# MerlinPCarson/WakeWord-Detection

Hardware: NVIDIA B200
Metric: audio_hours_per_sec (higher is better)
Workload: dtype f16x2->f32

## Files before the change

wakeword_detection_b200/csrc/wavenet_tc.cu:

```cuda
#include <string.h>

#include "wavenet_tc.cuh"

namespace wwb {


struct WnSmem {
  unsigned char U[WN_UBUF];
  float4 skip[8 * WN_ROWS];
  unsigned char W[WN_WST][WN_WBLK];
  WnHead head;
  uint64_t bar_gate[WN_NT], bar_rs[WN_NT], bar_det[WN_NT];
  uint64_t bar_u[WN_NT];
  uint64_t bar_dq[WN_NT];
  uint64_t bar_g[WN_NT];
  uint64_t wfull[WN_WST];
  uint32_t tmem_base;
  int zmax[2][WN_G][2];
  int zcnt[2];
};


#ifdef WWB_WN_DBG2
#define WN_DBG2(k, ev) do { if (P.dbg && blockIdx.x == 0 && grp == (int64_t)gridDim.x) P.dbg[WN_DBG_ROLES * 48 * 4 + 64 + (k) * 16 + (ev)] = clock64(); } while (0)
#else
#define WN_DBG2(k, ev) do { } while (0)
#endif
#ifdef WWB_TIMELINE
#define WN_DBG(role, k, ev) do { if (P.dbg && blockIdx.x == 0 && (grp == (int64_t)gridDim.x || grp == 2 * (int64_t)gridDim.x)) P.dbg[((role) * 48 + (k) + (grp == (int64_t)gridDim.x ? 0 : 24)) * 4 + (ev)] = clock64(); } while (0)
#else
#define WN_DBG(role, k, ev) do { } while (0)
#endif


__device__ __forceinline__ void epi_bar_sync() { asm volatile("bar.sync 1, %0;" ::"n"(WN_EPI_THREADS) : "memory"); }

#ifdef WWB_HANG_DEBUG
#define WN_SPIN_LIMIT (1u << 21)
#define WN_HANG_BASE 4096
__device__ __noinline__ void wn_hang(long long* dbg, int warp, int id, int hk, int hi, uint32_t n_u, uint32_t hx) {
  if (dbg && (threadIdx.x & 31) == 0) {
    long long* base = dbg + WN_HANG_BASE + ((long long)blockIdx.x * 32 + warp) * 8;
    base[0] = id; base[1] = hk; base[2] = hi; base[3] = n_u; base[4] = hx; base[5] = clock64();
  }
  asm volatile("exit;");
}
#define WN_BOUNDED(cond, id) do { uint32_t sp_ = 0; while (!(cond)) if (++sp_ > WN_SPIN_LIMIT) wn_hang(P.dbg, warp, id, hk, hi, n_u, hx); } while (0)
#define WN_MBAR_WAIT(bar, par, id) WN_BOUNDED(mbar_try_wait(bar, par), id)
#define WN_SPIN(bar, par, id) WN_BOUNDED(mbar_test_wait(bar, par), id)
#define WN_HSET(var, val) var = (val)
#else
#define WN_MBAR_WAIT(bar, par, id) mbar_wait(bar, par)
#define WN_SPIN(bar, par, id) mbar_spin(bar, par)
#define WN_HSET(var, val) do { } while (0)
#endif
__device__ __forceinline__ void mbar_spin(uint64_t* bar, uint32_t parity) {
#pragma unroll 1
  while (!mbar_test_wait(bar, parity)) { }
}
#define WN_WAIT_E(bar, par, id) WN_MBAR_WAIT(bar, par, id)
#ifndef WWB_WN_ISS_SUSPEND
#define WN_WAIT_I(bar, par, id) WN_SPIN(bar, par, id)
#else
#define WN_WAIT_I(bar, par, id) WN_MBAR_WAIT(bar, par, id)
#endif

__global__ void __launch_bounds__(WN_THREADS, 1) wavenet_tc_kernel(const WnTcParams P) {
  extern __shared__ __align__(128) unsigned char smem_raw[];
  WnSmem& sm = *reinterpret_cast<WnSmem*>(smem_raw);
  const int tid = threadIdx.x, lane = tid & 31;
  const int warp = __shfl_sync(0xffffffffu, tid >> 5, 0);
  const int64_t n_win = P.wm.n_win_dev ? (int64_t)*P.wm.n_win_dev : P.wm.n_win;
  const int64_t n_groups = P.stream_mode ? P.wm.n_streams * (int64_t)P.chunks_per_stream : (n_win + WN_G - 1) / WN_G;
  const int L = P.L;

  for (int i = tid; i < (int)(sizeof(sm.U) / 16); i += WN_THREADS) reinterpret_cast<uint4*>(sm.U)[i] = make_uint4(0, 0, 0, 0);
  for (int i = tid; i < (int)(sizeof(WnHead) / 16); i += WN_THREADS)
    reinterpret_cast<uint4*>(&sm.head)[i] = reinterpret_cast<const uint4*>(P.head)[i];
  if (tid < 2 * WN_G * 2) (&sm.zmax[0][0][0])[tid] = WN_KEY_NEG_INF;
  if (tid < 2) sm.zcnt[tid] = 0;
  if (tid == 0) {
    for (int i = 0; i < WN_NT; ++i) {
      mbar_init(&sm.bar_u[i], i == 0 ? 5 : 4); mbar_init(&sm.bar_g[i], 4); mbar_init(&sm.bar_gate[i], 1); mbar_init(&sm.bar_rs[i], 1);
      mbar_init(&sm.bar_det[i], 1); mbar_init(&sm.bar_dq[i], 4);
    }
    for (int s = 0; s < WN_WST; ++s) mbar_init(&sm.wfull[s], 1);
    mbar_fence_init();
  }
  if (warp == WN_EPI_WARPS) tmem_alloc(&sm.tmem_base, 512);
  fence_async_smem();
  fence_before_sync();
  __syncthreads();
  fence_after_sync();
  const uint32_t tmem = sm.tmem_base;
  const int nsplit = P.nsplit;
  const uint32_t idesc_gate = make_idesc_f16(128, 32), idesc_rs = make_idesc_f16(128, 48);

  if (warp < WN_EPI_WARPS) {
    const int tile = warp >> 2, q = warp & 3;
    const int o = tile * 128 + q * 32 + lane;
    const int R = P.rstride;
    const int t = o / R, w = o - t * R;
    const uint32_t tacc = tmem + tile * WN_TMEM_TILE;
    const uint32_t tbase = tacc + ((uint32_t)(q * 32) << 16);
    uint32_t n_gate = 0, n_rs = 0, n_u = 0;
#ifdef WWB_HANG_DEBUG
    int hk = -1, hi = tile; uint32_t hx = 0;
#endif
    unsigned char* const Urow = sm.U + (WN_PAD + o) * 16;
    float4* const sk = sm.skip + o;
    {
      uint32_t one[16];
#pragma unroll
      for (int i = 0; i < 16; ++i) one[i] = 0u;
      one[0] = 0x3c003c00u;
      tmem_st16(tmem + ((uint32_t)(q * 32) << 16) + WN_C_ONE, one);
      tmem_st_wait();
    }
    const u64 ZERO2 = pk(0.f, 0.f), ONE2 = pk(1.f, 1.f);
    const int jn = P.join[tile];
    const int src_slot = P.src_slot[tile];
    const bool stream_mode = P.stream_mode != 0;

    u64 x[8];
    bool valid = false, snap_out = false;
    int64_t b = 0;
    float* snap_dst = nullptr;
    auto fetch_state = [&](int64_t g) {
      bool vn = g < n_groups;
      int64_t row = 0;
      snap_out = false;
      if (stream_mode) {
        const int64_t s0 = g / P.chunks_per_stream;
        const int c = (int)(g - s0 * P.chunks_per_stream);
        const int f = c * WN_CHUNK_STEP + o;
        vn = vn && f < P.wm.ring;
        row = s0 * P.wm.ring + (vn ? f : 0);
        snap_out = vn && (c == 0 || o >= WN_CHUNK_WARM);
        snap_dst = P.snap + row * 4;
      } else {
        b = g * WN_G + w;
        vn = vn && (t < L) && (b < n_win);
        int64_t s0 = 0;
        int start = 0;
        if (vn) win_origin(P.wm, b, s0, start);
        int rr = start + (vn ? t : 0);
        if (rr >= P.wm.ring) rr -= P.wm.ring;
        row = s0 * P.wm.ring + rr;
      }
      valid = vn;
      if (src_slot >= 0) {
        const float4* p = reinterpret_cast<const float4*>(P.snap) + (int64_t)src_slot * (WN_SNAP_F / 4) * P.n_rows + row;
#pragma unroll
        for (int i = 0; i < 4; ++i) {
          const float4 v = vn ? __ldg(p + (int64_t)i * P.n_rows) : make_float4(0.f, 0.f, 0.f, 0.f);
          x[2 * i] = pk(v.x, v.y);
          x[2 * i + 1] = pk(v.z, v.w);
        }
#pragma unroll
        for (int i = 0; i < 8; ++i) sk[i * WN_ROWS] = vn ? __ldg(p + (int64_t)(4 + i) * P.n_rows) : make_float4(0.f, 0.f, 0.f, 0.f);
      } else {
        const float4* p = reinterpret_cast<const float4*>(P.x0) + row;
#pragma unroll
        for (int i = 0; i < 4; ++i) {
          const float4 v = vn ? __ldg(p + (int64_t)i * P.n_rows) : make_float4(0.f, 0.f, 0.f, 0.f);
          x[2 * i] = pk(v.x, v.y);
          x[2 * i + 1] = pk(v.z, v.w);
        }
#pragma unroll
        for (int i = 0; i < 8; ++i) sk[i * WN_ROWS] = make_float4(0.f, 0.f, 0.f, 0.f);
      }
    };
    auto put_start_state = [&]() {
      uint32_t ur[16];
#pragma unroll
      for (int i = 0; i < 8; ++i) split2(x[i], ur[i], ur[8 + i]);
      if (valid) {
        *reinterpret_cast<uint4*>(Urow) = make_uint4(ur[0], ur[1], ur[2], ur[3]);
        *reinterpret_cast<uint4*>(Urow + WN_PU) = make_uint4(ur[4], ur[5], ur[6], ur[7]);
        *reinterpret_cast<uint4*>(Urow + 2 * WN_PU) = make_uint4(ur[8], ur[9], ur[10], ur[11]);
        *reinterpret_cast<uint4*>(Urow + 3 * WN_PU) = make_uint4(ur[12], ur[13], ur[14], ur[15]);
      }
      tmem_st16(tbase + WN_C_U, ur);
      tmem_st_wait();
      fence_before_sync();
      fence_async_smem();
      __syncwarp();
      if (lane == 0) mbar_arrive(&sm.bar_u[tile]);
    };
    fetch_state(blockIdx.x);
    if ((int64_t)blockIdx.x < n_groups) put_start_state();
    for (int64_t grp = blockIdx.x; grp < n_groups; grp += gridDim.x, ++n_u) {
      const bool valid_g = valid;
      const bool snap_g = snap_out;
      float* const snap_g_dst = snap_dst;
      for (int k = jn; k < 24; ++k) {
        WN_HSET(hk, k);
        WN_WAIT_E(&sm.bar_gate[tile], n_gate & 1, 5);
        ++n_gate;
        fence_after_sync();
        if (q == 0 && lane == 0) WN_DBG(tile, k, 0);
        if (tile == 0 && q == 0 && lane == 0) WN_DBG2(k, 0);
        {
#pragma unroll
          for (int h8 = 0; h8 < 2; ++h8) {
            float v[16];
            tmem_ld16(tbase + h8 * 16, v);
            tmem_ld_wait();
            if (h8 == 0 && tile == 0 && q == 0 && lane == 0) WN_DBG2(k, 1);
            uint32_t gh[4], gl[4];
#pragma unroll
            for (int p = 0; p < 4; ++p) {
              const float a0 = v[2 * p], a1 = v[2 * p + 1], b0 = v[8 + 2 * p], b1 = v[8 + 2 * p + 1];
              const float ea0 = ex2_approx(fminf(a0, 30.f)), ea1 = ex2_approx(fminf(a1, 30.f));
              const float eb0 = ex2_approx(fminf(b0, 30.f)), eb1 = ex2_approx(fminf(b1, 30.f));
              const u64 tt = fadd2(pk(eb0, eb1), ONE2);
              float d0, d1;
              upk(ffma2(pk(ea0, ea1), tt, tt), d0, d1);
              const float rp = rcp_approx(d0 * d1);
              const float r0 = rp * d1, r1 = rp * d0;
              const u64 g = pk(fmaf(-ea0, r0, r0), fmaf(-ea1, r1, r1));
              split2(g, gh[p], gl[p]);
            }
            tmem_st4(tbase + WN_C_G + h8 * 4, gh);
            tmem_st4(tbase + WN_C_G + 8 + h8 * 4, gl);
          }
          if (tile == 0 && q == 0 && lane == 0) WN_DBG2(k, 2);
          tmem_st_wait();
          if (tile == 0 && q == 0 && lane == 0) WN_DBG2(k, 3);
        }
        fence_before_sync();
        if (q == 0 && lane == 0) WN_DBG(tile, k, 1);
        __syncwarp();
        if (lane == 0) mbar_arrive(&sm.bar_g[tile]);
        if (tile == 0 && q == 0 && lane == 0) WN_DBG2(k, 4);

        WN_WAIT_E(&sm.bar_rs[tile], n_rs & 1, 6);
        ++n_rs;
        fence_after_sync();
        if (q == 0 && lane == 0) WN_DBG(tile, k, 2);
        if (tile == 0 && q == 0 && lane == 0) WN_DBG2(k, 5);
        const bool last = (k == 23);
        if (!last) {
#pragma unroll
          for (int h8 = 0; h8 < 2; ++h8) {
            float r[8];
            tmem_ld8(tbase + WN_C_R + h8 * 8, r);
            tmem_ld_wait();
            uint32_t uh[4], ul[4];
#pragma unroll
            for (int p = 0; p < 4; ++p) {
              const int c = h8 * 4 + p;
              x[c] = add_relu2(x[c], pk(r[2 * p], r[2 * p + 1]));
              split2(x[c], uh[p], ul[p]);
            }
            if (valid_g) {
              *reinterpret_cast<uint4*>(Urow + h8 * WN_PU) = make_uint4(uh[0], uh[1], uh[2], uh[3]);
              *reinterpret_cast<uint4*>(Urow + (2 + h8) * WN_PU) = make_uint4(ul[0], ul[1], ul[2], ul[3]);
            }
            tmem_st4(tbase + WN_C_U + h8 * 4, uh);
            tmem_st4(tbase + WN_C_U + 8 + h8 * 4, ul);
          }
          if (tile == 0 && q == 0 && lane == 0) WN_DBG2(k, 6);
          tmem_st_wait();
          if (tile == 0 && q == 0 && lane == 0) WN_DBG2(k, 8);
          fence_before_sync();
          fence_async_smem();
          __syncwarp();
          if (lane == 0) mbar_arrive(&sm.bar_u[tile]);
          if (q == 0 && lane == 0) WN_DBG(tile, k, 3);
          if (tile == 0 && q == 0 && lane == 0) WN_DBG2(k, 9);
        }
#pragma unroll
        for (int h8 = 0; h8 < 4; ++h8) {
          float s[8];
          tmem_ld8(tbase + WN_C_R + 16 + h8 * 8, s);
          const float4 c0 = sk[(2 * h8) * WN_ROWS], c1 = sk[(2 * h8 + 1) * WN_ROWS];
          tmem_ld_wait();
          const u64 n0 = add_relu2(pk(c0.x, c0.y), pk(s[0], s[1])), n1 = add_relu2(pk(c0.z, c0.w), pk(s[2], s[3]));
          const u64 n2 = add_relu2(pk(c1.x, c1.y), pk(s[4], s[5])), n3 = add_relu2(pk(c1.z, c1.w), pk(s[6], s[7]));
          float4 o0, o1;
          upk(n0, o0.x, o0.y); upk(n1, o0.z, o0.w); upk(n2, o1.x, o1.y); upk(n3, o1.z, o1.w);
          sk[(2 * h8) * WN_ROWS] = o0;
          sk[(2 * h8 + 1) * WN_ROWS] = o1;
          if (last) {
            uint32_t eh[4], el[4];
            split2(relu2(n0), eh[0], el[0]); split2(relu2(n1), eh[1], el[1]);
            split2(relu2(n2), eh[2], el[2]); split2(relu2(n3), eh[3], el[3]);
            const uint32_t cx = tbase + (h8 < 2 ? WN_C_U : WN_C_G) + (h8 & 1) * 4;
            tmem_st4(cx, eh);
            tmem_st4(cx + 8, el);
          }
        }
        fence_before_sync();
        if (stream_mode) {
          const int sl = P.snap_slot[k];
          if (sl >= 0 && snap_g) {
            float4* dst = reinterpret_cast<float4*>(snap_g_dst) + (int64_t)sl * (WN_SNAP_F / 4) * P.n_rows;
#pragma unroll
            for (int i = 0; i < 4; ++i) {
              float a0, a1, a2, a3;
              upk(x[2 * i], a0, a1);
              upk(x[2 * i + 1], a2, a3);
              dst[(int64_t)i * P.n_rows] = make_float4(a0, a1, a2, a3);
            }
#pragma unroll
            for (int i = 0; i < 8; ++i) dst[(int64_t)(4 + i) * P.n_rows] = sk[i * WN_ROWS];
          }
        }
        if (last) {
          tmem_st_wait();
          fence_before_sync();
          __syncwarp();
          if (lane == 0) mbar_arrive(&sm.bar_dq[tile]);
          if (q == 0 && lane == 0) WN_DBG(tile, k, 3);
        }
      }

      if (P.enc_out && valid_g) {
        float4* dst = reinterpret_cast<float4*>(P.enc_out + ((grp * WN_G + w) * L + t) * 32);
#pragma unroll
        for (int n = 0; n < 8; ++n) dst[n] = sk[n * WN_ROWS];
      }
      if (tile == 0 && q == 0 && lane == 0) WN_DBG(WN_NT + 1, 20, 0);
      WN_HSET(hk, 24);
      fetch_state(grp + gridDim.x);
      WN_MBAR_WAIT(&sm.bar_det[tile], n_u & 1, 8);
      fence_after_sync();
      if (tile == 0 && q == 0 && lane == 0) WN_DBG(WN_NT + 1, 20, 1);
      float z0, z1;
      {
        u64 acc0[2] = {pk(0.f, 0.f), pk(0.f, 0.f)}, acc1[2] = {pk(0.f, 0.f), pk(0.f, 0.f)};
#pragma unroll
        for (int h8 = 0; h8 < 4; ++h8) {
          float d[8];
          tmem_ld8(tbase + WN_C_R + h8 * 8, d);
          tmem_ld_wait();
#pragma unroll
          for (int p = 0; p < 4; ++p) {
            const int c = h8 * 8 + 2 * p;
            const u64 e = relu2(fadd2(pk(d[2 * p], d[2 * p + 1]), pk(P.det1_b[c], P.det1_b[c + 1])));
            acc0[p & 1] = ffma2(pk(P.det2_w[c], P.det2_w[c + 1]), e, acc0[p & 1]);
            acc1[p & 1] = ffma2(pk(P.det2_w[32 + c], P.det2_w[32 + c + 1]), e, acc1[p & 1]);
          }
        }
        float fa, fb;
        upk(fadd2(acc0[0], acc0[1]), fa, fb);
        z0 = (fa + fb) + P.det2_b[0];
        upk(fadd2(acc1[0], acc1[1]), fa, fb);
        z1 = (fa + fb) + P.det2_b[1];
      }
      const int zp = (int)(n_u & 1);
      if (!stream_mode) {
#pragma unroll
        for (int dw = 0; dw < WN_G; ++dw) {
          const bool mine = valid_g && (w == dw);
          const unsigned m = __ballot_sync(0xffffffffu, mine);
          if (m) {
            const int k0 = __reduce_max_sync(0xffffffffu, mine ? f2key(z0) : WN_KEY_NEG_INF);
            const int k1 = __reduce_max_sync(0xffffffffu, mine ? f2key(z1) : WN_KEY_NEG_INF);
            if (lane == 0) {
              atomicMax(&sm.zmax[zp][dw][0], k0);
              atomicMax(&sm.zmax[zp][dw][1], k1);
            }
          }
        }
        if (tile == 0 && q == 0 && lane == 0) WN_DBG(WN_NT + 1, 20, 2);
        if (lane == 0) {
          __threadfence_block();
          if (atomicAdd(&sm.zcnt[zp], 1) == WN_EPI_WARPS - 1) {
            __threadfence_block();
            for (int dw = 0; dw < WN_G; ++dw) {
              const int64_t bb = grp * WN_G + dw;
              const float a0 = key2f(sm.zmax[zp][dw][0]), a1 = key2f(sm.zmax[zp][dw][1]);
              sm.zmax[zp][dw][0] = WN_KEY_NEG_INF;
              sm.zmax[zp][dw][1] = WN_KEY_NEG_INF;
              if (bb < n_win) {
                const float m = fmaxf(a0, a1);
                const float e0 = expf(a0 - m), e1 = expf(a1 - m), sden = e0 + e1;
                if (P.det_out) { P.det_out[bb * 2] = e0 / sden; P.det_out[bb * 2 + 1] = e1 / sden; }
                if (P.post) P.post[bb] = e1 / sden;
              }
            }
            sm.zcnt[zp] = 0;
          }
        }
        __syncwarp();
      }
      put_start_state();
      if (tile == 0 && q == 0 && lane == 0) WN_DBG(WN_NT + 1, 20, 3);
    }
  } else if (warp == WN_EPI_WARPS) {
    uint32_t n_u = 0;
#ifdef WWB_HANG_DEBUG
    int hk = -1, hi = -1; uint32_t hx = 0;
#endif
    const uint64_t dU = make_desc(smem_u32(sm.U), WN_PU, 128);
    const uint64_t dWg = make_desc(smem_u32(sm.W[0]), 512, 128);
    const uint64_t dBg = make_desc(smem_u32(sm.W[0]) + WN_OFF_GBIAS, 512, 128);
    const uint64_t dH = make_desc(smem_u32(sm.head.det1_B), 512, 128);
    uint32_t my_groups = 0;
    for (int64_t grp = blockIdx.x; grp < n_groups; grp += gridDim.x) ++my_groups;
    const uint32_t total_loads = my_groups * 24;
    for (uint32_t n = 0; n < (uint32_t)WN_WST && n < total_loads; ++n)
      if (lane == 0) {
        mbar_arrive_expect_tx(&sm.wfull[n], WN_WBLK);
        bulk_g2s(sm.W[n], P.wblob + (size_t)n * WN_WBLK, WN_WBLK, &sm.wfull[n]);
      }
    uint32_t n_w = 0;
    uint32_t cu[WN_NT];
#pragma unroll
    for (int i = 0; i < WN_NT; ++i) cu[i] = 0;
    const uint32_t rs3 = (uint32_t)P.rstride;
    for (int64_t grp = blockIdx.x; grp < n_groups; grp += gridDim.x, ++n_u) {
      for (int k = 0; k < 24; ++k, ++n_w) {
        WN_MBAR_WAIT(&sm.wfull[n_w % WN_WST], (n_w / WN_WST) & 1, 1);
        const uint32_t d = (uint32_t)P.dil[k] * rs3;
        const uint64_t wofs = (uint64_t)((n_w % WN_WST) * (WN_WBLK >> 4));
        const uint64_t b0 = dWg + wofs, bb = dBg + wofs;
#pragma unroll
        for (int i = 0; i < WN_NT; ++i) {
          if (k < P.join[i]) continue;
          WN_HSET(hk, k); WN_HSET(hi, i);
          if (i == 1) WN_DBG(WN_NT + 1, k, 0);
          if (i == 0 && lane == 0) WN_DBG2(k, 10);
          WN_WAIT_I(&sm.bar_u[i], cu[i] & 1, 2);
          ++cu[i];
          if (i == 0 && lane == 0) WN_DBG2(k, 11);
          if (i == 1) WN_DBG(WN_NT + 1, k, 1);
          fence_after_sync();
          if (elect_one()) {
            const uint32_t tacc = tmem + i * WN_TMEM_TILE;
            const uint64_t a0 = dU + (uint64_t)(WN_PAD + i * 128 - 2 * d), a1 = dU + (uint64_t)(WN_PAD + i * 128 - d);
            const uint64_t lo_a = (uint64_t)((2 * WN_PU) >> 4), lo_b = (uint64_t)(3072 >> 4);
            mma_f16_ss(tacc, a0, b0, idesc_gate, false);
            if (nsplit == 3) {
              mma_f16_ss(tacc, a0 + lo_a, b0, idesc_gate, true);
              mma_f16_ss(tacc, a0, b0 + lo_b, idesc_gate, true);
            }
            mma_f16_ss(tacc, a1, b0 + 64, idesc_gate, true);
            if (nsplit == 3) {
              mma_f16_ss(tacc, a1 + lo_a, b0 + 64, idesc_gate, true);
              mma_f16_ss(tacc, a1, b0 + 64 + lo_b, idesc_gate, true);
            }
            mma_f16_ts(tacc, tacc + WN_C_U, b0 + 128, idesc_gate, true);
            if (nsplit == 3) {
              mma_f16_ts(tacc, tacc + WN_C_U + 8, b0 + 128, idesc_gate, true);
              mma_f16_ts(tacc, tacc + WN_C_U, b0 + 128 + lo_b, idesc_gate, true);
            }
            mma_f16_ts(tacc, tmem + WN_C_ONE, bb, idesc_gate, true);
            mma_commit(&sm.bar_gate[i]);
            if (i == 0) WN_DBG2(k, 12);
            if (i == 0) WN_DBG(WN_NT, k, 0);
            if (i == WN_NT - 1) WN_DBG(WN_NT, k, 1);
          }
          __syncwarp();
          if (i == 1) WN_DBG(WN_NT + 1, k, 2);
        }
        auto refill = [&](uint32_t m) {
          const uint32_t nl = m + WN_WST;
          if (nl < total_loads && lane == 0) {
            mbar_arrive_expect_tx(&sm.wfull[nl % WN_WST], WN_WBLK);
            bulk_g2s(sm.W[nl % WN_WST], P.wblob + (size_t)(nl % 24) * WN_WBLK, WN_WBLK, &sm.wfull[nl % WN_WST]);
          }
        };
        if (n_w >= 1) refill(n_w - 1);
      }
#pragma unroll
      for (int i = 0; i < WN_NT; ++i) {
        WN_MBAR_WAIT(&sm.bar_dq[i], n_u & 1, 9);
        fence_after_sync();
        if (elect_one()) {
          const uint32_t tacc = tmem + i * WN_TMEM_TILE;
#pragma unroll
          for (int kk = 0; kk < 2; ++kk) {
            const uint32_t ta = tacc + (kk == 0 ? WN_C_U : WN_C_G);
            const uint64_t bh = dH + (uint64_t)((kk * 2 * 512) >> 4), bl = bh + (uint64_t)(2048 >> 4);
            mma_f16_ts(tacc + WN_C_R, ta, bh, idesc_gate, kk != 0);
            if (nsplit == 3) {
              mma_f16_ts(tacc + WN_C_R, ta + 8, bh, idesc_gate, true);
              mma_f16_ts(tacc + WN_C_R, ta, bl, idesc_gate, true);
            }
          }
          mma_commit(&sm.bar_det[i]);
        }
        __syncwarp();
      }
    }
  } else {
    uint32_t n_u = 0, n_w = 0;
#ifdef WWB_HANG_DEBUG
    int hk = -1, hi = -1; uint32_t hx = 0;
#endif
    const uint64_t dWr = make_desc(smem_u32(sm.W[0]) + WN_GATE_B, 768, 128);
    const uint64_t dBr = make_desc(smem_u32(sm.W[0]) + WN_OFF_RBIAS, 768, 128);
    const uint32_t ones = tmem + WN_C_ONE;
    uint32_t cg[WN_NT];
#pragma unroll
    for (int i = 0; i < WN_NT; ++i) cg[i] = 0;
    auto store_pad = [&](const unsigned char* chunk) {
      const uint4* c4 = reinterpret_cast<const uint4*>(chunk);
      const uint4 c0 = c4[0], c1 = c4[1], c2 = c4[2], c3 = c4[3];
#pragma unroll
      for (int r = lane; r < WN_PAD; r += 32) {
        unsigned char* up = sm.U + r * 16;
        *reinterpret_cast<uint4*>(up) = c0;
        *reinterpret_cast<uint4*>(up + WN_PU) = c1;
        *reinterpret_cast<uint4*>(up + 2 * WN_PU) = c2;
        *reinterpret_cast<uint4*>(up + 3 * WN_PU) = c3;
      }
      fence_async_smem();
      __syncwarp();
      if (lane == 0) mbar_arrive(&sm.bar_u[0]);
    };
    if ((int64_t)blockIdx.x < n_groups) store_pad(sm.head.pad0);
    for (int64_t grp = blockIdx.x; grp < n_groups; grp += gridDim.x, ++n_u) {
      for (int k = 0; k < 24; ++k, ++n_w) {
        const uint64_t wofs = (uint64_t)((n_w % WN_WST) * (WN_WBLK >> 4));
        const uint64_t bh = dWr + wofs, bb = dBr + wofs, lo_b = (uint64_t)(1536 >> 4);
        WN_MBAR_WAIT(&sm.wfull[n_w % WN_WST], (n_w / WN_WST) & 1, 11);
#pragma unroll
        for (int i = 0; i < WN_NT; ++i) {
          if (k < P.join[i]) continue;
          WN_HSET(hk, k); WN_HSET(hi, i);
          if (i == 3) WN_DBG(WN_NT + 2, k, 0);
          WN_WAIT_I(&sm.bar_g[i], cg[i] & 1, 10);
          if (i < WN_NT - 1 && k >= P.join[i + 1]) WN_WAIT_I(&sm.bar_gate[i + 1], cg[i + 1] & 1, 3);
          ++cg[i];
          if (i == 0 && lane == 0) WN_DBG2(k, 13);
          if (i == 3) WN_DBG(WN_NT + 2, k, 1);
          fence_after_sync();
          if (elect_one()) {
            const uint32_t tacc = tmem + i * WN_TMEM_TILE;
            mma_f16_ts(tacc + WN_C_R, tacc + WN_C_G, bh, idesc_rs, false);
            if (nsplit == 3) {
              mma_f16_ts(tacc + WN_C_R, tacc + WN_C_G + 8, bh, idesc_rs, true);
              mma_f16_ts(tacc + WN_C_R, tacc + WN_C_G, bh + lo_b, idesc_rs, true);
            }
            mma_f16_ts(tacc + WN_C_R, ones, bb, idesc_rs, true);
            mma_commit(&sm.bar_rs[i]);
            if (i == 0) WN_DBG2(k, 14);
            if (i == 0) WN_DBG(WN_NT, k, 2);
            if (i == WN_NT - 1) WN_DBG(WN_NT, k, 3);
          }
          __syncwarp();
          if (i == 0)
            store_pad(k < 23 ? sm.W[n_w % WN_WST] + WN_OFF_F32 + 320 : sm.head.pad0);
          if (i == 3) WN_DBG(WN_NT + 2, k, 2);
        }
      }
    }
  }
  fence_before_sync();
  __syncthreads();
  if (warp == WN_EPI_WARPS) tmem_dealloc(tmem, 512);
}

static double gate_scale(int n) { return n < 16 ? -2.8853900817779268 : -1.4426950408889634; }
static int gate_col(int n) { const int c = n & 15; return (c >> 3) * 16 + (n >> 4) * 8 + (c & 7); }

static void put_split(std::vector<unsigned char>& buf, size_t hi_off, size_t lo_off, float x, bool split) {
  __half h = __float2half_rn(x);
  __half l = split ? __float2half_rn(x - __half2float(h)) : __float2half_rn(0.f);
  memcpy(&buf[hi_off], &h, 2);
  memcpy(&buf[lo_off], &l, 2);
}

static bool put_pad_rows(std::vector<unsigned char>& out, size_t off, const float* mul, const float* add) {
  for (int c = 0; c < 16; ++c) {
    if (mul[c] == 0.f) return false;
    const size_t o = off + (size_t)(c / 8) * 16 + (c % 8) * 2;
    put_split(out, o, o + 32, (float)(-(double)add[c] / (double)mul[c]), true);
  }
  return true;
}

std::vector<unsigned char> wavenet_pack_blocks(const float* gate_w, const float* gate_b, const float* rs_w,
                                               const float* rs_b, const float* bn_mul, const float* bn_add,
                                               const int* dilation) {
  std::vector<unsigned char> out((size_t)24 * WN_WBLK, 0);
  for (int b = 0; b < 24; ++b) {
    const size_t base = (size_t)b * WN_WBLK;
    for (int k = 0; k < 48; ++k)
      for (int n = 0; n < 32; ++n) {
        const int c = k / 8, e = k % 8;
        const size_t off = base + ((size_t)c * 32 + gate_col(n)) * 16 + e * 2;
        put_split(out, off, off + 3072, (float)((double)gate_w[((size_t)b * 48 + k) * 32 + n] * (double)bn_mul[b * 16 + k % 16] * gate_scale(n)), true);
      }
    for (int k = 0; k < 16; ++k)
      for (int n = 0; n < 48; ++n) {
        const int c = k / 8, e = k % 8;
        const size_t off = base + WN_GATE_B + ((size_t)c * 48 + n) * 16 + e * 2;
        put_split(out, off, off + 1536, rs_w[((size_t)b * 16 + k) * 48 + n], true);
      }
    float f[113] = {0};
    f[112] = (float)dilation[b];
    memcpy(&out[base + WN_OFF_F32], f, sizeof(f));
    if (b < 23 && !put_pad_rows(out, base + WN_OFF_F32 + 320, bn_mul + (b + 1) * 16, bn_add + (b + 1) * 16)) return {};
    for (int n = 0; n < 32; ++n) {
      const size_t off = base + WN_OFF_GBIAS + (size_t)gate_col(n) * 16;
      double bsum = gate_b[b * 32 + n];
      for (int k = 0; k < 48; ++k) bsum += (double)gate_w[((size_t)b * 48 + k) * 32 + n] * (double)bn_add[b * 16 + k % 16];
      put_split(out, off, off + 2, (float)(bsum * gate_scale(n)), true);
    }
    for (int n = 0; n < 48; ++n) {
      const size_t off = base + WN_OFF_RBIAS + (size_t)n * 16;
      put_split(out, off, off + 2, rs_b[b * 48 + n], true);
    }
  }
  return out;
}

std::vector<unsigned char> wavenet_pack_head(const float* bn_mul0, const float* bn_add0, const float* det1_w_nk,
                                             const float* det1_b, const float* det2_w, const float* det2_b) {
  std::vector<unsigned char> out(sizeof(WnHead), 0);
  WnHead* h = reinterpret_cast<WnHead*>(out.data());
  if (!put_pad_rows(out, offsetof(WnHead, pad0), bn_mul0, bn_add0)) return {};
  h = reinterpret_cast<WnHead*>(out.data());
  memcpy(h->det1_b, det1_b, sizeof(h->det1_b));
  memcpy(h->det2_w, det2_w, sizeof(h->det2_w));
  memcpy(h->det2_b, det2_b, sizeof(h->det2_b));
  const size_t boff = offsetof(WnHead, det1_B);
  for (int n = 0; n < 32; ++n)
    for (int k = 0; k < 32; ++k) {
      const int c = k / 8, e = k % 8;
      const size_t off = boff + ((size_t)c * 32 + n) * 16 + e * 2;
      put_split(out, off, off + 2048, det1_w_nk[n * 32 + k], true);
    }
  return out;
}

__global__ void __launch_bounds__(256) wn_input_kernel(const float* __restrict__ mel, const float* __restrict__ w_kc,
                                                       const float* __restrict__ b, float* __restrict__ x0, int64_t n_rows) {
  __shared__ float ws[kMel * 16];
  __shared__ float bs[16];
  for (int i = threadIdx.x; i < kMel * 16; i += 256) ws[i] = w_kc[i];
  if (threadIdx.x < 16) bs[threadIdx.x] = b[threadIdx.x];
  __syncthreads();
  const int c4 = threadIdx.x & 3;
  for (int64_t row = (int64_t)blockIdx.x * 64 + (threadIdx.x >> 2); row < n_rows; row += (int64_t)gridDim.x * 64) {
    const float4* m4 = reinterpret_cast<const float4*>(mel + row * kMel);
    float a0 = bs[4 * c4], a1 = bs[4 * c4 + 1], a2 = bs[4 * c4 + 2], a3 = bs[4 * c4 + 3];
#pragma unroll
    for (int k4 = 0; k4 < kMel / 4; ++k4) {
      const float4 m = __ldg(m4 + k4);
      const float mv[4] = {m.x, m.y, m.z, m.w};
#pragma unroll
      for (int e = 0; e < 4; ++e) {
        const float4 wv = *reinterpret_cast<const float4*>(ws + (4 * k4 + e) * 16 + 4 * c4);
        a0 = fmaf(wv.x, mv[e], a0); a1 = fmaf(wv.y, mv[e], a1); a2 = fmaf(wv.z, mv[e], a2); a3 = fmaf(wv.w, mv[e], a3);
      }
    }
    reinterpret_cast<float4*>(x0)[(int64_t)c4 * n_rows + row] = make_float4(fmaxf(a0, 0.f), fmaxf(a1, 0.f), fmaxf(a2, 0.f), fmaxf(a3, 0.f));
  }
}

struct WnSharePlan {
  int join[WN_NT], src_slot[WN_NT], snap_slot[24], n_slots;
};
static WnSharePlan wn_share_plan(const int* dil, int L) {
  WnSharePlan g;
  for (int k = 0; k < 24; ++k) g.snap_slot[k] = -1;
  g.n_slots = 0;
  int D[24], acc = 0;
  for (int k = 0; k < 24; ++k) { acc += 2 * dil[k]; D[k] = acc; }
  for (int i = 0; i < WN_NT; ++i) {
    const int tmin = (i * 128) / WN_G;
    int j = 23;
    for (int k = 0; k < 24; ++k)
      if (D[k] > tmin) { j = k; break; }
    if (tmin >= L) j = 23;
    g.join[i] = j;
    g.src_slot[i] = -1;
    if (j > 0 && tmin < L) {
      if (g.snap_slot[j - 1] < 0) g.snap_slot[j - 1] = g.n_slots++;
      g.src_slot[i] = g.snap_slot[j - 1];
    }
  }
  return g;
}

int wavenet_tc_posteriors(wwb_ctx* ctx, const WinMap& wm, float* enc_out, float* det_out, float* post,
                          cudaStream_t st) {
  if (wm.n_win == 0) return WWB_OK;
  if (ctx->L > WN_MAXT) return fail(ctx, WWB_ERR_ARG, "tensor-core WaveNet path supports windows up to 182 frames");
  const int64_t n_rows = wm.n_streams * (int64_t)wm.ring;
  void* x0;
  int rc = workspace(ctx, 1, (size_t)std::max<int64_t>(n_rows, 1) * 16 * sizeof(float), &x0);
  if (rc) return rc;
  wn_input_kernel<<<(unsigned)std::min<int64_t>((n_rows + 63) / 64, (int64_t)ctx->sm_count * 8), 256, 0, st>>>(
      wm.mel, ctx->wn.in_w, ctx->wn.in_b, (float*)x0, n_rows);
  WWB_CHECK_LAUNCH(ctx);
  WnTcParams P;
  memset(&P, 0, sizeof(P));
  P.x0 = (const float*)x0;
  P.wm = wm;
  P.wblob = ctx->wn.tc_blocks;
  P.head = reinterpret_cast<const WnHead*>(ctx->wn.tc_head);
  P.L = ctx->L;
  P.nsplit = ctx->precision == WWB_PREC_TC ? 3 : 1;
  for (int b = 0; b < 24; ++b) { P.dil[b] = ctx->wn.dilation[b]; P.snap_slot[b] = -1; }
  for (int i = 0; i < WN_NT; ++i) { P.join[i] = 0; P.src_slot[i] = -1; }
  memcpy(P.det1_b, ctx->wn.h_det1_b, sizeof(P.det1_b));
  memcpy(P.det2_w, ctx->wn.h_det2_w, sizeof(P.det2_w));
  memcpy(P.det2_b, ctx->wn.h_det2_b, sizeof(P.det2_b));
  P.n_rows = n_rows;
  P.dbg = reinterpret_cast<long long*>(ctx->debug_buf);
  const size_t smem = sizeof(WnSmem) + 128;
  WWB_CUDA(ctx, cudaFuncSetAttribute(wavenet_tc_kernel, cudaFuncAttributeMaxDynamicSharedMemorySize, (int)smem));

  const char* no_share = getenv("WWB_WN_NO_SHARE");
  const bool share = !wm.win_stream && !wm.n_win_dev && wm.b0 == 0 && wm.win_per_stream >= 8 && wm.hop < ctx->L &&
                     !(no_share && no_share[0] == '1');
  if (share) {
    const WnSharePlan g = wn_share_plan(ctx->wn.dilation, ctx->L);
    if (g.n_slots > 0) {
      void* snap;
      if ((rc = workspace(ctx, 2, (size_t)g.n_slots * n_rows * WN_SNAP_F * sizeof(float), &snap))) return rc;
      WnTcParams S = P;
      S.stream_mode = 1;
      S.rstride = 1;
      S.chunks_per_stream = wm.ring <= WN_ROWS ? 1 : 1 + (wm.ring - WN_ROWS + WN_CHUNK_STEP - 1) / WN_CHUNK_STEP;
      S.snap = (float*)snap;
      for (int b = 0; b < 24; ++b) S.snap_slot[b] = g.snap_slot[b];
      S.enc_out = S.det_out = S.post = nullptr;
#ifndef WWB_HANG_DEBUG
      S.dbg = nullptr;
#endif
      const int64_t n_chunks = wm.n_streams * (int64_t)S.chunks_per_stream;
      wavenet_tc_kernel<<<(unsigned)std::min<int64_t>(n_chunks, ctx->sm_count), WN_THREADS, smem, st>>>(S);
      WWB_CHECK_LAUNCH(ctx);
      P.snap = (float*)snap;
      for (int i = 0; i < WN_NT; ++i) { P.join[i] = g.join[i]; P.src_slot[i] = g.src_slot[i]; }
    }
  }
  P.rstride = WN_G;
  P.enc_out = enc_out; P.det_out = det_out; P.post = post;
  const int64_t n_groups = (wm.n_win + WN_G - 1) / WN_G;
  const unsigned grid = (unsigned)std::min<int64_t>(n_groups, ctx->sm_count);
  wavenet_tc_kernel<<<grid, WN_THREADS, smem, st>>>(P);
  WWB_CHECK_LAUNCH(ctx);
  return WWB_OK;
}

}
```

wakeword_detection_b200/csrc/wavenet_tc.cuh:

```cuda
#pragma once
#include "common.cuh"
#include "tc_common.cuh"

namespace wwb {

using namespace tc;

constexpr int WN_G = 4;
constexpr int WN_NT = 6;
constexpr int WN_ROWS = WN_NT * 128;
constexpr int WN_PAD = 16 * WN_G;
constexpr int WN_UROWS = WN_ROWS + WN_PAD;
constexpr int WN_MAXT = 182;
constexpr int WN_CHUNK_WARM = 180;
constexpr int WN_CHUNK_STEP = WN_ROWS - WN_CHUNK_WARM;
constexpr int WN_SNAP_F = 48;
constexpr int WN_PU = WN_UROWS * 16;
constexpr int WN_UBUF = 4 * WN_PU;
constexpr int WN_EPI_WARPS = WN_NT * 4;
constexpr int WN_EPI_THREADS = WN_EPI_WARPS * 32;
constexpr int WN_THREADS = (WN_EPI_WARPS + 2) * 32;
constexpr int WN_GATE_B = 6144, WN_RS_B = 3072;
constexpr int WN_F32_B = 512;
constexpr int WN_GBIAS_B = 1024, WN_RBIAS_B = 1536;
constexpr int WN_OFF_F32 = WN_GATE_B + WN_RS_B, WN_OFF_GBIAS = WN_OFF_F32 + WN_F32_B, WN_OFF_RBIAS = WN_OFF_GBIAS + WN_GBIAS_B;
constexpr int WN_WBLK = WN_OFF_RBIAS + WN_RBIAS_B;
constexpr int WN_WST = 5;
constexpr int WN_TMEM_TILE = 80;
constexpr int WN_C_G = 0;
constexpr int WN_C_R = 16;
constexpr int WN_C_U = 64;
constexpr int WN_DBG_ROLES = WN_NT + 3;
constexpr int WN_C_ONE = WN_NT * WN_TMEM_TILE;


struct WnHead {
  unsigned char pad0[64];
  unsigned char rsv_[64];
  float det1_b[32];
  float det2_w[2 * 32];
  float det2_b[2];
  float pad_[2];
  unsigned char det1_B[2 * 4 * 32 * 16];
};

struct WnTcParams {
  WinMap wm;
  const unsigned char* wblob;
  const WnHead* head;
  const float* x0;
  int L;
  int nsplit;
  int dil[24];
  int rstride;
  int stream_mode;
  int chunks_per_stream;
  int join[WN_NT];
  int src_slot[WN_NT];
  int snap_slot[24];
  float det1_b[32], det2_w[64], det2_b[2];
  float* snap;
  int64_t n_rows;
  float* enc_out;
  float* det_out;
  float* post;
  long long* dbg;
};

__device__ __forceinline__ float ex2_approx(float x) {
  float y;
  asm("ex2.approx.ftz.f32 %0, %1;" : "=f"(y) : "f"(x));
  return y;
}
__device__ __forceinline__ float rcp_approx(float x) {
  float y;
  asm("rcp.approx.ftz.f32 %0, %1;" : "=f"(y) : "f"(x));
  return y;
}
__device__ __forceinline__ u64 relu2(u64 v) { float a, b; upk(v, a, b); return pk(fmaxf(a, 0.f), fmaxf(b, 0.f)); }
__device__ __forceinline__ u64 add_relu2(u64 acc, u64 v) {
  float a, b;
  upk(v, a, b);
  return ffma2(fadd2(v, pk(fabsf(a), fabsf(b))), pk(0.5f, 0.5f), acc);
}

__device__ __forceinline__ void tmem_ld8(uint32_t taddr, float (&v)[8]) {
  uint32_t r[8];
  asm volatile("tcgen05.ld.sync.aligned.32x32b.x8.b32 {%0,%1,%2,%3,%4,%5,%6,%7}, [%8];"
               : "=r"(r[0]), "=r"(r[1]), "=r"(r[2]), "=r"(r[3]), "=r"(r[4]), "=r"(r[5]), "=r"(r[6]), "=r"(r[7])
               : "r"(taddr));
#pragma unroll
  for (int i = 0; i < 8; ++i) v[i] = __uint_as_float(r[i]);
}
__device__ __forceinline__ int f2key(float v) { const int i = __float_as_int(v); return i ^ ((i >> 31) & 0x7fffffff); }
__device__ __forceinline__ float key2f(int k) { return __int_as_float(k ^ ((k >> 31) & 0x7fffffff)); }
constexpr int WN_KEY_NEG_INF = (int)0x807fffff;

}
```

Before: 91.01.

## Split WaveNet into early-layer dense-group phase and late-layer handoff phase

Templates the WaveNet tensor-core kernel on group size, tile count, end layer and handoff input. When sharing is possible, the first five dilated layers run in a separate launch that packs 16 windows per CTA over a short receptive field. That launch writes intermediate state to a handoff buffer, and the main kernel resumes from layer kb, so the per-window row padding wasted in the small-dilation layers is avoided. The cost is extra launches, a large global handoff buffer and its round trip through memory, plus chunked processing of windows.

```diff
diff --git a/wakeword_detection_b200/csrc/wavenet_tc.cu b/wakeword_detection_b200/csrc/wavenet_tc.cu
--- a/wakeword_detection_b200/csrc/wavenet_tc.cu
+++ b/wakeword_detection_b200/csrc/wavenet_tc.cu
@@ -1,22 +1,37 @@
 #include <string.h>
 
+#include <atomic>
+
 #include "wavenet_tc.cuh"
 
 namespace wwb {
 
 
+template <int G, int NT>
+struct WnGeo {
+  static constexpr int ROWS = NT * 128;
+  static constexpr int PAD = 16 * G;
+  static constexpr int PU = (ROWS + PAD) * 16;
+  static constexpr int EPI_WARPS = NT * 4;
+  static constexpr int THREADS = (EPI_WARPS + 2) * 32;
+  static constexpr int C_ONE = NT * WN_TMEM_TILE;
+};
+
+template <int G, int NT>
 struct WnSmem {
-  unsigned char U[WN_UBUF];
-  float4 skip[8 * WN_ROWS];
+  using Geo = WnGeo<G, NT>;
+  unsigned char U[4 * Geo::PU];
+  float4 skip[8 * Geo::ROWS];
   unsigned char W[WN_WST][WN_WBLK];
   WnHead head;
-  uint64_t bar_gate[WN_NT], bar_rs[WN_NT], bar_det[WN_NT];
-  uint64_t bar_u[WN_NT];
-  uint64_t bar_dq[WN_NT];
-  uint64_t bar_g[WN_NT];
+  uint4 pad_first[4];
+  uint64_t bar_gate[NT], bar_rs[NT], bar_det[NT];
+  uint64_t bar_u[NT];
+  uint64_t bar_dq[NT];
+  uint64_t bar_g[NT];
   uint64_t wfull[WN_WST];
   uint32_t tmem_base;
-  int zmax[2][WN_G][2];
+  int zmax[2][G][2];
   int zcnt[2];
 };
 
@@ -32,8 +47,6 @@
 #define WN_DBG(role, k, ev) do { } while (0)
 #endif
 
-
-__device__ __forceinline__ void epi_bar_sync() { asm volatile("bar.sync 1, %0;" ::"n"(WN_EPI_THREADS) : "memory"); }
 
 #ifdef WWB_HANG_DEBUG
 #define WN_SPIN_LIMIT (1u << 21)
@@ -65,29 +78,35 @@
 #define WN_WAIT_I(bar, par, id) WN_MBAR_WAIT(bar, par, id)
 #endif
 
-__global__ void __launch_bounds__(WN_THREADS, 1) wavenet_tc_kernel(const WnTcParams P) {
+template <int G, int NT, int KE, bool HIN>
+__global__ void __launch_bounds__(WnGeo<G, NT>::THREADS, 1) wavenet_tc_kernel(const WnTcParams P) {
+  using Geo = WnGeo<G, NT>;
+  constexpr int ROWS = Geo::ROWS, PAD = Geo::PAD, PU = Geo::PU, EPI_WARPS = Geo::EPI_WARPS, THREADS = Geo::THREADS;
+  constexpr bool DETECT = KE == 24;
   extern __shared__ __align__(128) unsigned char smem_raw[];
-  WnSmem& sm = *reinterpret_cast<WnSmem*>(smem_raw);
+  WnSmem<G, NT>& sm = *reinterpret_cast<WnSmem<G, NT>*>(smem_raw);
   const int tid = threadIdx.x, lane = tid & 31;
   const int warp = __shfl_sync(0xffffffffu, tid >> 5, 0);
   const int64_t n_win = P.wm.n_win_dev ? (int64_t)*P.wm.n_win_dev : P.wm.n_win;
-  const int64_t n_groups = P.stream_mode ? P.wm.n_streams * (int64_t)P.chunks_per_stream : (n_win + WN_G - 1) / WN_G;
+  const int64_t n_groups = DETECT && P.stream_mode ? P.wm.n_streams * (int64_t)P.chunks_per_stream : (n_win + G - 1) / G;
   const int L = P.L;
 
-  for (int i = tid; i < (int)(sizeof(sm.U) / 16); i += WN_THREADS) reinterpret_cast<uint4*>(sm.U)[i] = make_uint4(0, 0, 0, 0);
-  for (int i = tid; i < (int)(sizeof(WnHead) / 16); i += WN_THREADS)
+  for (int i = tid; i < (int)(sizeof(sm.U) / 16); i += THREADS) reinterpret_cast<uint4*>(sm.U)[i] = make_uint4(0, 0, 0, 0);
+  for (int i = tid; i < (int)(sizeof(WnHead) / 16); i += THREADS)
     reinterpret_cast<uint4*>(&sm.head)[i] = reinterpret_cast<const uint4*>(P.head)[i];
-  if (tid < 2 * WN_G * 2) (&sm.zmax[0][0][0])[tid] = WN_KEY_NEG_INF;
+  if (tid < 4)
+    sm.pad_first[tid] = reinterpret_cast<const uint4*>(P.kb == 0 ? P.head->pad0 : P.wblob + (size_t)(P.kb - 1) * WN_WBLK + WN_OFF_F32 + 320)[tid];
+  if (tid < 2 * G * 2) (&sm.zmax[0][0][0])[tid] = WN_KEY_NEG_INF;
   if (tid < 2) sm.zcnt[tid] = 0;
   if (tid == 0) {
-    for (int i = 0; i < WN_NT; ++i) {
+    for (int i = 0; i < NT; ++i) {
       mbar_init(&sm.bar_u[i], i == 0 ? 5 : 4); mbar_init(&sm.bar_g[i], 4); mbar_init(&sm.bar_gate[i], 1); mbar_init(&sm.bar_rs[i], 1);
       mbar_init(&sm.bar_det[i], 1); mbar_init(&sm.bar_dq[i], 4);
     }
     for (int s = 0; s < WN_WST; ++s) mbar_init(&sm.wfull[s], 1);
     mbar_fence_init();
   }
-  if (warp == WN_EPI_WARPS) tmem_alloc(&sm.tmem_base, 512);
+  if (warp == EPI_WARPS) tmem_alloc(&sm.tmem_base, 512);
   fence_async_smem();
   fence_before_sync();
   __syncthreads();
@@ -96,7 +115,7 @@
   const int nsplit = P.nsplit;
   const uint32_t idesc_gate = make_idesc_f16(128, 32), idesc_rs = make_idesc_f16(128, 48);
 
-  if (warp < WN_EPI_WARPS) {
+  if (warp < EPI_WARPS) {
     const int tile = warp >> 2, q = warp & 3;
     const int o = tile * 128 + q * 32 + lane;
     const int R = P.rstride;
@@ -107,20 +126,20 @@
 #ifdef WWB_HANG_DEBUG
     int hk = -1, hi = tile; uint32_t hx = 0;
 #endif
-    unsigned char* const Urow = sm.U + (WN_PAD + o) * 16;
+    unsigned char* const Urow = sm.U + (PAD + o) * 16;
     float4* const sk = sm.skip + o;
     {
       uint32_t one[16];
 #pragma unroll
       for (int i = 0; i < 16; ++i) one[i] = 0u;
       one[0] = 0x3c003c00u;
-      tmem_st16(tmem + ((uint32_t)(q * 32) << 16) + WN_C_ONE, one);
+      tmem_st16(tmem + ((uint32_t)(q * 32) << 16) + Geo::C_ONE, one);
       tmem_st_wait();
     }
     const u64 ZERO2 = pk(0.f, 0.f), ONE2 = pk(1.f, 1.f);
     const int jn = P.join[tile];
     const int src_slot = P.src_slot[tile];
-    const bool stream_mode = P.stream_mode != 0;
+    const bool stream_mode = DETECT && P.stream_mode != 0;
 
     u64 x[8];
     bool valid = false, snap_out = false;
@@ -139,7 +158,7 @@
         snap_out = vn && (c == 0 || o >= WN_CHUNK_WARM);
         snap_dst = P.snap + row * 4;
       } else {
-        b = g * WN_G + w;
+        b = g * G + w;
         vn = vn && (t < L) && (b < n_win);
         int64_t s0 = 0;
         int start = 0;
@@ -151,6 +170,21 @@
       valid = vn;
       if (src_slot >= 0) {
         const float4* p = reinterpret_cast<const float4*>(P.snap) + (int64_t)src_slot * (WN_SNAP_F / 4) * P.n_rows + row;
+        int64_t ps = P.n_rows;
+        if (HIN && t < P.hand_rows) {
+          p = reinterpret_cast<const float4*>(P.hand) + ((b / WN_GE) * P.hand_rows + t) * WN_GE + b % WN_GE;
+          ps = P.n_hand;
+        }
+#pragma unroll
+        for (int i = 0; i < 4; ++i) {
+          const float4 v = vn ? __ldg(p + (int64_t)i * ps) : make_float4(0.f, 0.f, 0.f, 0.f);
+          x[2 * i] = pk(v.x, v.y);
+          x[2 * i + 1] = pk(v.z, v.w);
+        }
+#pragma unroll
+        for (int i = 0; i < 8; ++i) sk[i * ROWS] = vn ? __ldg(p + (int64_t)(4 + i) * ps) : make_float4(0.f, 0.f, 0.f, 0.f);
+      } else {
+        const float4* p = reinterpret_cast<const float4*>(P.x0) + row;
 #pragma unroll
         for (int i = 0; i < 4; ++i) {
           const float4 v = vn ? __ldg(p + (int64_t)i * P.n_rows) : make_float4(0.f, 0.f, 0.f, 0.f);
@@ -158,17 +192,7 @@
           x[2 * i + 1] = pk(v.z, v.w);
         }
 #pragma unroll
-        for (int i = 0; i < 8; ++i) sk[i * WN_ROWS] = vn ? __ldg(p + (int64_t)(4 + i) * P.n_rows) : make_float4(0.f, 0.f, 0.f, 0.f);
-      } else {
-        const float4* p = reinterpret_cast<const float4*>(P.x0) + row;
-#pragma unroll
-        for (int i = 0; i < 4; ++i) {
-          const float4 v = vn ? __ldg(p + (int64_t)i * P.n_rows) : make_float4(0.f, 0.f, 0.f, 0.f);
-          x[2 * i] = pk(v.x, v.y);
-          x[2 * i + 1] = pk(v.z, v.w);
-        }
-#pragma unroll
-        for (int i = 0; i < 8; ++i) sk[i * WN_ROWS] = make_float4(0.f, 0.f, 0.f, 0.f);
+        for (int i = 0; i < 8; ++i) sk[i * ROWS] = make_float4(0.f, 0.f, 0.f, 0.f);
       }
     };
     auto put_start_state = [&]() {
@@ -177,9 +201,9 @@
       for (int i = 0; i < 8; ++i) split2(x[i], ur[i], ur[8 + i]);
       if (valid) {
         *reinterpret_cast<uint4*>(Urow) = make_uint4(ur[0], ur[1], ur[2], ur[3]);
-        *reinterpret_cast<uint4*>(Urow + WN_PU) = make_uint4(ur[4], ur[5], ur[6], ur[7]);
-        *reinterpret_cast<uint4*>(Urow + 2 * WN_PU) = make_uint4(ur[8], ur[9], ur[10], ur[11]);
-        *reinterpret_cast<uint4*>(Urow + 3 * WN_PU) = make_uint4(ur[12], ur[13], ur[14], ur[15]);
+        *reinterpret_cast<uint4*>(Urow + PU) = make_uint4(ur[4], ur[5], ur[6], ur[7]);
+        *reinterpret_cast<uint4*>(Urow + 2 * PU) = make_uint4(ur[8], ur[9], ur[10], ur[11]);
+        *reinterpret_cast<uint4*>(Urow + 3 * PU) = make_uint4(ur[12], ur[13], ur[14], ur[15]);
       }
       tmem_st16(tbase + WN_C_U, ur);
       tmem_st_wait();
@@ -194,7 +218,7 @@
       const bool valid_g = valid;
       const bool snap_g = snap_out;
       float* const snap_g_dst = snap_dst;
-      for (int k = jn; k < 24; ++k) {
+      for (int k = jn; k < KE; ++k) {
         WN_HSET(hk, k);
         WN_WAIT_E(&sm.bar_gate[tile], n_gate & 1, 5);
         ++n_gate;
@@ -240,8 +264,8 @@
         fence_after_sync();
         if (q == 0 && lane == 0) WN_DBG(tile, k, 2);
         if (tile == 0 && q == 0 && lane == 0) WN_DBG2(k, 5);
-        const bool last = (k == 23);
-        if (!last) {
+        const bool last = (k == KE - 1);
+        if (!(DETECT && last)) {
 #pragma unroll
           for (int h8 = 0; h8 < 2; ++h8) {
             float r[8];
@@ -254,36 +278,40 @@
               x[c] = add_relu2(x[c], pk(r[2 * p], r[2 * p + 1]));
               split2(x[c], uh[p], ul[p]);
             }
-            if (valid_g) {
-              *reinterpret_cast<uint4*>(Urow + h8 * WN_PU) = make_uint4(uh[0], uh[1], uh[2], uh[3]);
-              *reinterpret_cast<uint4*>(Urow + (2 + h8) * WN_PU) = make_uint4(ul[0], ul[1], ul[2], ul[3]);
-            }
-            tmem_st4(tbase + WN_C_U + h8 * 4, uh);
-            tmem_st4(tbase + WN_C_U + 8 + h8 * 4, ul);
-          }
-          if (tile == 0 && q == 0 && lane == 0) WN_DBG2(k, 6);
-          tmem_st_wait();
-          if (tile == 0 && q == 0 && lane == 0) WN_DBG2(k, 8);
-          fence_before_sync();
-          fence_async_smem();
-          __syncwarp();
-          if (lane == 0) mbar_arrive(&sm.bar_u[tile]);
-          if (q == 0 && lane == 0) WN_DBG(tile, k, 3);
-          if (tile == 0 && q == 0 && lane == 0) WN_DBG2(k, 9);
+            if (!last) {
+              if (valid_g) {
+                *reinterpret_cast<uint4*>(Urow + h8 * PU) = make_uint4(uh[0], uh[1], uh[2], uh[3]);
+                *reinterpret_cast<uint4*>(Urow + (2 + h8) * PU) = make_uint4(ul[0], ul[1], ul[2], ul[3]);
+              }
+              tmem_st4(tbase + WN_C_U + h8 * 4, uh);
+              tmem_st4(tbase + WN_C_U + 8 + h8 * 4, ul);
+            }
+          }
+          if (!last) {
+            if (tile == 0 && q == 0 && lane == 0) WN_DBG2(k, 6);
+            tmem_st_wait();
+            if (tile == 0 && q == 0 && lane == 0) WN_DBG2(k, 8);
+            fence_before_sync();
+            fence_async_smem();
+            __syncwarp();
+            if (lane == 0) mbar_arrive(&sm.bar_u[tile]);
+            if (q == 0 && lane == 0) WN_DBG(tile, k, 3);
+            if (tile == 0 && q == 0 && lane == 0) WN_DBG2(k, 9);
+          }
         }
 #pragma unroll
         for (int h8 = 0; h8 < 4; ++h8) {
           float s[8];
           tmem_ld8(tbase + WN_C_R + 16 + h8 * 8, s);
-          const float4 c0 = sk[(2 * h8) * WN_ROWS], c1 = sk[(2 * h8 + 1) * WN_ROWS];
+          const float4 c0 = sk[(2 * h8) * ROWS], c1 = sk[(2 * h8 + 1) * ROWS];
           tmem_ld_wait();
           const u64 n0 = add_relu2(pk(c0.x, c0.y), pk(s[0], s[1])), n1 = add_relu2(pk(c0.z, c0.w), pk(s[2], s[3]));
           const u64 n2 = add_relu2(pk(c1.x, c1.y), pk(s[4], s[5])), n3 = add_relu2(pk(c1.z, c1.w), pk(s[6], s[7]));
           float4 o0, o1;
           upk(n0, o0.x, o0.y); upk(n1, o0.z, o0.w); upk(n2, o1.x, o1.y); upk(n3, o1.z, o1.w);
-          sk[(2 * h8) * WN_ROWS] = o0;
-          sk[(2 * h8 + 1) * WN_ROWS] = o1;
-          if (last) {
+          sk[(2 * h8) * ROWS] = o0;
+          sk[(2 * h8 + 1) * ROWS] = o1;
+          if (DETECT && last) {
             uint32_t eh[4], el[4];
             split2(relu2(n0), eh[0], el[0]); split2(relu2(n1), eh[1], el[1]);
             split2(relu2(n2), eh[2], el[2]); split2(relu2(n3), eh[3], el[3]);
@@ -305,7 +333,7 @@
               dst[(int64_t)i * P.n_rows] = make_float4(a0, a1, a2, a3);
             }
 #pragma unroll
-            for (int i = 0; i < 8; ++i) dst[(int64_t)(4 + i) * P.n_rows] = sk[i * WN_ROWS];
+            for (int i = 0; i < 8; ++i) dst[(int64_t)(4 + i) * P.n_rows] = sk[i * ROWS];
           }
         }
         if (last) {
@@ -317,10 +345,27 @@
         }
       }
 
+      if constexpr (!DETECT) {
+        if (valid_g && t < P.hand_rows) {
+          float4* dst = reinterpret_cast<float4*>(P.hand) + grp * P.hand_rows * G + o;
+#pragma unroll
+          for (int i = 0; i < 4; ++i) {
+            float a0, a1, a2, a3;
+            upk(x[2 * i], a0, a1);
+            upk(x[2 * i + 1], a2, a3);
+            dst[(int64_t)i * P.n_hand] = make_float4(a0, a1, a2, a3);
+          }
+#pragma unroll
+          for (int i = 0; i < 8; ++i) dst[(int64_t)(4 + i) * P.n_hand] = sk[i * ROWS];
+        }
+        fetch_state(grp + gridDim.x);
+        put_start_state();
+        continue;
+      }
       if (P.enc_out && valid_g) {
-        float4* dst = reinterpret_cast<float4*>(P.enc_out + ((grp * WN_G + w) * L + t) * 32);
-#pragma unroll
-        for (int n = 0; n < 8; ++n) dst[n] = sk[n * WN_ROWS];
+        float4* dst = reinterpret_cast<float4*>(P.enc_out + ((grp * G + w) * L + t) * 32);
+#pragma unroll
+        for (int n = 0; n < 8; ++n) dst[n] = sk[n * ROWS];
       }
       if (tile == 0 && q == 0 && lane == 0) WN_DBG(WN_NT + 1, 20, 0);
       WN_HSET(hk, 24);
@@ -353,7 +398,7 @@
       const int zp = (int)(n_u & 1);
       if (!stream_mode) {
 #pragma unroll
-        for (int dw = 0; dw < WN_G; ++dw) {
+        for (int dw = 0; dw < G; ++dw) {
           const bool mine = valid_g && (w == dw);
           const unsigned m = __ballot_sync(0xffffffffu, mine);
           if (m) {
@@ -368,10 +413,10 @@
         if (tile == 0 && q == 0 && lane == 0) WN_DBG(WN_NT + 1, 20, 2);
         if (lane == 0) {
           __threadfence_block();
-          if (atomicAdd(&sm.zcnt[zp], 1) == WN_EPI_WARPS - 1) {
+          if (atomicAdd(&sm.zcnt[zp], 1) == EPI_WARPS - 1) {
             __threadfence_block();
-            for (int dw = 0; dw < WN_G; ++dw) {
-              const int64_t bb = grp * WN_G + dw;
+            for (int dw = 0; dw < G; ++dw) {
+              const int64_t bb = grp * G + dw;
               const float a0 = key2f(sm.zmax[zp][dw][0]), a1 = key2f(sm.zmax[zp][dw][1]);
               sm.zmax[zp][dw][0] = WN_KEY_NEG_INF;
               sm.zmax[zp][dw][1] = WN_KEY_NEG_INF;
@@ -390,36 +435,38 @@
       put_start_state();
       if (tile == 0 && q == 0 && lane == 0) WN_DBG(WN_NT + 1, 20, 3);
     }
-  } else if (warp == WN_EPI_WARPS) {
+  } else if (warp == EPI_WARPS) {
     uint32_t n_u = 0;
 #ifdef WWB_HANG_DEBUG
     int hk = -1, hi = -1; uint32_t hx = 0;
 #endif
-    const uint64_t dU = make_desc(smem_u32(sm.U), WN_PU, 128);
+    const uint64_t dU = make_desc(smem_u32(sm.U), PU, 128);
     const uint64_t dWg = make_desc(smem_u32(sm.W[0]), 512, 128);
     const uint64_t dBg = make_desc(smem_u32(sm.W[0]) + WN_OFF_GBIAS, 512, 128);
     const uint64_t dH = make_desc(smem_u32(sm.head.det1_B), 512, 128);
     uint32_t my_groups = 0;
     for (int64_t grp = blockIdx.x; grp < n_groups; grp += gridDim.x) ++my_groups;
-    const uint32_t total_loads = my_groups * 24;
+    const int kb = P.kb;
+    const uint32_t nblk = (uint32_t)(KE - kb);
+    const uint32_t total_loads = my_groups * nblk;
     for (uint32_t n = 0; n < (uint32_t)WN_WST && n < total_loads; ++n)
       if (lane == 0) {
         mbar_arrive_expect_tx(&sm.wfull[n], WN_WBLK);
-        bulk_g2s(sm.W[n], P.wblob + (size_t)n * WN_WBLK, WN_WBLK, &sm.wfull[n]);
+        bulk_g2s(sm.W[n], P.wblob + (size_t)(kb + n % nblk) * WN_WBLK, WN_WBLK, &sm.wfull[n]);
       }
     uint32_t n_w = 0;
-    uint32_t cu[WN_NT];
-#pragma unroll
-    for (int i = 0; i < WN_NT; ++i) cu[i] = 0;
+    uint32_t cu[NT];
+#pragma unroll
+    for (int i = 0; i < NT; ++i) cu[i] = 0;
     const uint32_t rs3 = (uint32_t)P.rstride;
     for (int64_t grp = blockIdx.x; grp < n_groups; grp += gridDim.x, ++n_u) {
-      for (int k = 0; k < 24; ++k, ++n_w) {
+      for (int k = kb; k < KE; ++k, ++n_w) {
         WN_MBAR_WAIT(&sm.wfull[n_w % WN_WST], (n_w / WN_WST) & 1, 1);
         const uint32_t d = (uint32_t)P.dil[k] * rs3;
         const uint64_t wofs = (uint64_t)((n_w % WN_WST) * (WN_WBLK >> 4));
         const uint64_t b0 = dWg + wofs, bb = dBg + wofs;
 #pragma unroll
-        for (int i = 0; i < WN_NT; ++i) {
+        for (int i = 0; i < NT; ++i) {
           if (k < P.join[i]) continue;
           WN_HSET(hk, k); WN_HSET(hi, i);
           if (i == 1) WN_DBG(WN_NT + 1, k, 0);
@@ -431,8 +478,8 @@
           fence_after_sync();
           if (elect_one()) {
             const uint32_t tacc = tmem + i * WN_TMEM_TILE;
-            const uint64_t a0 = dU + (uint64_t)(WN_PAD + i * 128 - 2 * d), a1 = dU + (uint64_t)(WN_PAD + i * 128 - d);
-            const uint64_t lo_a = (uint64_t)((2 * WN_PU) >> 4), lo_b = (uint64_t)(3072 >> 4);
+            const uint64_t a0 = dU + (uint64_t)(PAD + i * 128 - 2 * d), a1 = dU + (uint64_t)(PAD + i * 128 - d);
+            const uint64_t lo_a = (uint64_t)((2 * PU) >> 4), lo_b = (uint64_t)(3072 >> 4);
             mma_f16_ss(tacc, a0, b0, idesc_gate, false);
             if (nsplit == 3) {
               mma_f16_ss(tacc, a0 + lo_a, b0, idesc_gate, true);
@@ -448,26 +495,29 @@
               mma_f16_ts(tacc, tacc + WN_C_U + 8, b0 + 128, idesc_gate, true);
               mma_f16_ts(tacc, tacc + WN_C_U, b0 + 128 + lo_b, idesc_gate, true);
             }
-            mma_f16_ts(tacc, tmem + WN_C_ONE, bb, idesc_gate, true);
+            mma_f16_ts(tacc, tmem + Geo::C_ONE, bb, idesc_gate, true);
             mma_commit(&sm.bar_gate[i]);
             if (i == 0) WN_DBG2(k, 12);
             if (i == 0) WN_DBG(WN_NT, k, 0);
-            if (i == WN_NT - 1) WN_DBG(WN_NT, k, 1);
+            if (i == NT - 1) WN_DBG(WN_NT, k, 1);
           }
           __syncwarp();
           if (i == 1) WN_DBG(WN_NT + 1, k, 2);
         }
+        if (!DETECT && k == kb && n_u > 0)
+#pragma unroll
+          for (int i = 0; i < NT; ++i) WN_MBAR_WAIT(&sm.bar_dq[i], (n_u - 1) & 1, 9);
         auto refill = [&](uint32_t m) {
           const uint32_t nl = m + WN_WST;
           if (nl < total_loads && lane == 0) {
             mbar_arrive_expect_tx(&sm.wfull[nl % WN_WST], WN_WBLK);
-            bulk_g2s(sm.W[nl % WN_WST], P.wblob + (size_t)(nl % 24) * WN_WBLK, WN_WBLK, &sm.wfull[nl % WN_WST]);
+            bulk_g2s(sm.W[nl % WN_WST], P.wblob + (size_t)(kb + nl % nblk) * WN_WBLK, WN_WBLK, &sm.wfull[nl % WN_WST]);
           }
         };
         if (n_w >= 1) refill(n_w - 1);
       }
 #pragma unroll
-      for (int i = 0; i < WN_NT; ++i) {
+      for (int i = 0; i < (DETECT ? NT : 0); ++i) {
         WN_MBAR_WAIT(&sm.bar_dq[i], n_u & 1, 9);
         fence_after_sync();
         if (elect_one()) {
@@ -494,38 +544,39 @@
 #endif
     const uint64_t dWr = make_desc(smem_u32(sm.W[0]) + WN_GATE_B, 768, 128);
     const uint64_t dBr = make_desc(smem_u32(sm.W[0]) + WN_OFF_RBIAS, 768, 128);
-    const uint32_t ones = tmem + WN_C_ONE;
-    uint32_t cg[WN_NT];
-#pragma unroll
-    for (int i = 0; i < WN_NT; ++i) cg[i] = 0;
+    const uint32_t ones = tmem + Geo::C_ONE;
+    uint32_t cg[NT];
+#pragma unroll
+    for (int i = 0; i < NT; ++i) cg[i] = 0;
     auto store_pad = [&](const unsigned char* chunk) {
       const uint4* c4 = reinterpret_cast<const uint4*>(chunk);
       const uint4 c0 = c4[0], c1 = c4[1], c2 = c4[2], c3 = c4[3];
 #pragma unroll
-      for (int r = lane; r < WN_PAD; r += 32) {
+      for (int r = lane; r < PAD; r += 32) {
         unsigned char* up = sm.U + r * 16;
         *reinterpret_cast<uint4*>(up) = c0;
-        *reinterpret_cast<uint4*>(up + WN_PU) = c1;
-        *reinterpret_cast<uint4*>(up + 2 * WN_PU) = c2;
-        *reinterpret_cast<uint4*>(up + 3 * WN_PU) = c3;
+        *reinterpret_cast<uint4*>(up + PU) = c1;
+        *reinterpret_cast<uint4*>(up + 2 * PU) = c2;
+        *reinterpret_cast<uint4*>(up + 3 * PU) = c3;
       }
       fence_async_smem();
       __syncwarp();
       if (lane == 0) mbar_arrive(&sm.bar_u[0]);
     };
-    if ((int64_t)blockIdx.x < n_groups) store_pad(sm.head.pad0);
+    const unsigned char* const pad_first = reinterpret_cast<const unsigned char*>(sm.pad_first);
+    if ((int64_t)blockIdx.x < n_groups) store_pad(pad_first);
     for (int64_t grp = blockIdx.x; grp < n_groups; grp += gridDim.x, ++n_u) {
-      for (int k = 0; k < 24; ++k, ++n_w) {
+      for (int k = P.kb; k < KE; ++k, ++n_w) {
         const uint64_t wofs = (uint64_t)((n_w % WN_WST) * (WN_WBLK >> 4));
         const uint64_t bh = dWr + wofs, bb = dBr + wofs, lo_b = (uint64_t)(1536 >> 4);
         WN_MBAR_WAIT(&sm.wfull[n_w % WN_WST], (n_w / WN_WST) & 1, 11);
 #pragma unroll
-        for (int i = 0; i < WN_NT; ++i) {
+        for (int i = 0; i < NT; ++i) {
           if (k < P.join[i]) continue;
           WN_HSET(hk, k); WN_HSET(hi, i);
           if (i == 3) WN_DBG(WN_NT + 2, k, 0);
           WN_WAIT_I(&sm.bar_g[i], cg[i] & 1, 10);
-          if (i < WN_NT - 1 && k >= P.join[i + 1]) WN_WAIT_I(&sm.bar_gate[i + 1], cg[i + 1] & 1, 3);
+          if (i < NT - 1 && k >= P.join[i + 1]) WN_WAIT_I(&sm.bar_gate[i + 1], cg[i + 1] & 1, 3);
           ++cg[i];
           if (i == 0 && lane == 0) WN_DBG2(k, 13);
           if (i == 3) WN_DBG(WN_NT + 2, k, 1);
@@ -541,11 +592,11 @@
             mma_commit(&sm.bar_rs[i]);
             if (i == 0) WN_DBG2(k, 14);
             if (i == 0) WN_DBG(WN_NT, k, 2);
-            if (i == WN_NT - 1) WN_DBG(WN_NT, k, 3);
+            if (i == NT - 1) WN_DBG(WN_NT, k, 3);
           }
           __syncwarp();
           if (i == 0)
-            store_pad(k < 23 ? sm.W[n_w % WN_WST] + WN_OFF_F32 + 320 : sm.head.pad0);
+            store_pad(k < KE - 1 ? sm.W[n_w % WN_WST] + WN_OFF_F32 + 320 : pad_first);
           if (i == 3) WN_DBG(WN_NT + 2, k, 2);
         }
       }
@@ -553,7 +604,7 @@
   }
   fence_before_sync();
   __syncthreads();
-  if (warp == WN_EPI_WARPS) tmem_dealloc(tmem, 512);
+  if (warp == EPI_WARPS) tmem_dealloc(tmem, 512);
 }
 
 static double gate_scale(int n) { return n < 16 ? -2.8853900817779268 : -1.4426950408889634; }
@@ -655,29 +706,35 @@
   }
 }
 
-struct WnSharePlan {
-  int join[WN_NT], src_slot[WN_NT], snap_slot[24], n_slots;
-};
-static WnSharePlan wn_share_plan(const int* dil, int L) {
-  WnSharePlan g;
-  for (int k = 0; k < 24; ++k) g.snap_slot[k] = -1;
-  g.n_slots = 0;
-  int D[24], acc = 0;
-  for (int k = 0; k < 24; ++k) { acc += 2 * dil[k]; D[k] = acc; }
-  for (int i = 0; i < WN_NT; ++i) {
-    const int tmin = (i * 128) / WN_G;
-    int j = 23;
-    for (int k = 0; k < 24; ++k)
+static void wn_share_plan(const int* D, int L, int g, int nt, int kb, int ke, int* join, int* src_slot, int* snap_slot,
+                          int& n_slots) {
+  for (int i = 0; i < nt; ++i) {
+    const int tmin = (i * 128) / g;
+    int j = ke - 1;
+    for (int k = kb; k < ke; ++k)
       if (D[k] > tmin) { j = k; break; }
-    if (tmin >= L) j = 23;
-    g.join[i] = j;
-    g.src_slot[i] = -1;
+    if (tmin >= L) j = ke - 1;
+    join[i] = j;
+    src_slot[i] = -1;
     if (j > 0 && tmin < L) {
-      if (g.snap_slot[j - 1] < 0) g.snap_slot[j - 1] = g.n_slots++;
-      g.src_slot[i] = g.snap_slot[j - 1];
-    }
-  }
-  return g;
+      if (snap_slot[j - 1] < 0) snap_slot[j - 1] = n_slots++;
+      src_slot[i] = snap_slot[j - 1];
+    }
+  }
+}
+
+template <int G, int NT, int KE, bool HIN>
+static int wn_launch(wwb_ctx* ctx, const WnTcParams& P, int64_t n_groups, cudaStream_t st) {
+  const size_t smem = sizeof(WnSmem<G, NT>) + 128;
+  static std::atomic<uint64_t> attr_set{0};
+  const uint64_t bit = 1ull << (ctx->device & 63);
+  if (!(attr_set.load() & bit)) {
+    WWB_CUDA(ctx, cudaFuncSetAttribute(wavenet_tc_kernel<G, NT, KE, HIN>, cudaFuncAttributeMaxDynamicSharedMemorySize, (int)smem));
+    attr_set.fetch_or(bit);
+  }
+  wavenet_tc_kernel<G, NT, KE, HIN><<<(unsigned)std::min<int64_t>(n_groups, ctx->sm_count), WnGeo<G, NT>::THREADS, smem, st>>>(P);
+  WWB_CHECK_LAUNCH(ctx);
+  return WWB_OK;
 }
 
 int wavenet_tc_posteriors(wwb_ctx* ctx, const WinMap& wm, float* enc_out, float* det_out, float* post,
@@ -706,40 +763,69 @@
   memcpy(P.det2_b, ctx->wn.h_det2_b, sizeof(P.det2_b));
   P.n_rows = n_rows;
   P.dbg = reinterpret_cast<long long*>(ctx->debug_buf);
-  const size_t smem = sizeof(WnSmem) + 128;
-  WWB_CUDA(ctx, cudaFuncSetAttribute(wavenet_tc_kernel, cudaFuncAttributeMaxDynamicSharedMemorySize, (int)smem));
+  P.rstride = WN_G;
+  P.enc_out = enc_out; P.det_out = det_out; P.post = post;
 
   const char* no_share = getenv("WWB_WN_NO_SHARE");
   const bool share = !wm.win_stream && !wm.n_win_dev && wm.b0 == 0 && wm.win_per_stream >= 8 && wm.hop < ctx->L &&
                      !(no_share && no_share[0] == '1');
-  if (share) {
-    const WnSharePlan g = wn_share_plan(ctx->wn.dilation, ctx->L);
-    if (g.n_slots > 0) {
-      void* snap;
-      if ((rc = workspace(ctx, 2, (size_t)g.n_slots * n_rows * WN_SNAP_F * sizeof(float), &snap))) return rc;
-      WnTcParams S = P;
-      S.stream_mode = 1;
-      S.rstride = 1;
-      S.chunks_per_stream = wm.ring <= WN_ROWS ? 1 : 1 + (wm.ring - WN_ROWS + WN_CHUNK_STEP - 1) / WN_CHUNK_STEP;
-      S.snap = (float*)snap;
-      for (int b = 0; b < 24; ++b) S.snap_slot[b] = g.snap_slot[b];
-      S.enc_out = S.det_out = S.post = nullptr;
+  if (!share) return wn_launch<WN_G, WN_NT, 24, false>(ctx, P, (wm.n_win + WN_G - 1) / WN_G, st);
+
+  int D[24], acc = 0;
+  for (int k = 0; k < 24; ++k) { acc += 2 * ctx->wn.dilation[k]; D[k] = acc; }
+  const int S = WN_KE;
+  const char* one_phase = getenv("WWB_WN_ONE_PHASE");
+  const bool two = D[S - 1] * WN_GE <= WN_NTE * 128 && !enc_out && !det_out && !(one_phase && one_phase[0] == '1');
+  int n_slots = 0;
+  WnTcParams E = P;
+  if (two) {
+    P.kb = S;
+    P.hand_rows = D[S - 1];
+    E.rstride = WN_GE;
+    E.enc_out = E.det_out = E.post = nullptr;
+    E.dbg = nullptr;
+    wn_share_plan(D, ctx->L, WN_GE, WN_NTE, 0, S, E.join, E.src_slot, P.snap_slot, n_slots);
+  }
+  wn_share_plan(D, ctx->L, WN_G, WN_NT, P.kb, 24, P.join, P.src_slot, P.snap_slot, n_slots);
+  void* snap = nullptr;
+  if (n_slots > 0) {
+    if ((rc = workspace(ctx, 2, (size_t)n_slots * n_rows * WN_SNAP_F * sizeof(float), &snap))) return rc;
+    WnTcParams S1 = P;
+    S1.kb = 0;
+    S1.hand_rows = 0;
+    S1.stream_mode = 1;
+    S1.rstride = 1;
+    S1.chunks_per_stream = wm.ring <= WN_ROWS ? 1 : 1 + (wm.ring - WN_ROWS + WN_CHUNK_STEP - 1) / WN_CHUNK_STEP;
+    S1.snap = (float*)snap;
+    for (int i = 0; i < WN_NT; ++i) { S1.join[i] = 0; S1.src_slot[i] = -1; }
+    S1.enc_out = S1.det_out = S1.post = nullptr;
 #ifndef WWB_HANG_DEBUG
-      S.dbg = nullptr;
+    S1.dbg = nullptr;
 #endif
-      const int64_t n_chunks = wm.n_streams * (int64_t)S.chunks_per_stream;
-      wavenet_tc_kernel<<<(unsigned)std::min<int64_t>(n_chunks, ctx->sm_count), WN_THREADS, smem, st>>>(S);
-      WWB_CHECK_LAUNCH(ctx);
-      P.snap = (float*)snap;
-      for (int i = 0; i < WN_NT; ++i) { P.join[i] = g.join[i]; P.src_slot[i] = g.src_slot[i]; }
-    }
-  }
-  P.rstride = WN_G;
-  P.enc_out = enc_out; P.det_out = det_out; P.post = post;
-  const int64_t n_groups = (wm.n_win + WN_G - 1) / WN_G;
-  const unsigned grid = (unsigned)std::min<int64_t>(n_groups, ctx->sm_count);
-  wavenet_tc_kernel<<<grid, WN_THREADS, smem, st>>>(P);
-  WWB_CHECK_LAUNCH(ctx);
+    if ((rc = wn_launch<WN_G, WN_NT, 24, false>(ctx, S1, wm.n_streams * (int64_t)S1.chunks_per_stream, st))) return rc;
+  }
+  P.snap = E.snap = (float*)snap;
+  for (int b = 0; b < 24; ++b) P.snap_slot[b] = E.snap_slot[b] = -1;
+  if (!two) return wn_launch<WN_G, WN_NT, 24, false>(ctx, P, (wm.n_win + WN_G - 1) / WN_G, st);
+
+  const int64_t wave = (int64_t)WN_GE * ctx->sm_count;
+  const int64_t row_bytes = (int64_t)WN_SNAP_F * sizeof(float) * P.hand_rows;
+  const int64_t chunk = std::min<int64_t>(std::max<int64_t>(1, WN_HAND_MAX_BYTES / (wave * row_bytes)) * wave,
+                                          (wm.n_win + WN_GE - 1) / WN_GE * WN_GE);
+  const int64_t n_hand = chunk * P.hand_rows;
+  void* hand;
+  if ((rc = workspace(ctx, 6, (size_t)n_hand * WN_SNAP_F * sizeof(float), &hand))) return rc;
+  P.hand = E.hand = (float*)hand;
+  P.n_hand = E.n_hand = n_hand;
+  E.hand_rows = P.hand_rows;
+  for (int64_t c0 = 0; c0 < wm.n_win; c0 += chunk) {
+    const int64_t nw = std::min(chunk, wm.n_win - c0);
+    E.wm.b0 = P.wm.b0 = c0;
+    E.wm.n_win = P.wm.n_win = nw;
+    P.post = post ? post + c0 : nullptr;
+    if ((rc = wn_launch<WN_GE, WN_NTE, WN_KE, false>(ctx, E, (nw + WN_GE - 1) / WN_GE, st))) return rc;
+    if ((rc = wn_launch<WN_G, WN_NT, 24, true>(ctx, P, (nw + WN_G - 1) / WN_G, st))) return rc;
+  }
   return WWB_OK;
 }
 
diff --git a/wakeword_detection_b200/csrc/wavenet_tc.cuh b/wakeword_detection_b200/csrc/wavenet_tc.cuh
--- a/wakeword_detection_b200/csrc/wavenet_tc.cuh
+++ b/wakeword_detection_b200/csrc/wavenet_tc.cuh
@@ -9,17 +9,10 @@
 constexpr int WN_G = 4;
 constexpr int WN_NT = 6;
 constexpr int WN_ROWS = WN_NT * 128;
-constexpr int WN_PAD = 16 * WN_G;
-constexpr int WN_UROWS = WN_ROWS + WN_PAD;
 constexpr int WN_MAXT = 182;
 constexpr int WN_CHUNK_WARM = 180;
 constexpr int WN_CHUNK_STEP = WN_ROWS - WN_CHUNK_WARM;
 constexpr int WN_SNAP_F = 48;
-constexpr int WN_PU = WN_UROWS * 16;
-constexpr int WN_UBUF = 4 * WN_PU;
-constexpr int WN_EPI_WARPS = WN_NT * 4;
-constexpr int WN_EPI_THREADS = WN_EPI_WARPS * 32;
-constexpr int WN_THREADS = (WN_EPI_WARPS + 2) * 32;
 constexpr int WN_GATE_B = 6144, WN_RS_B = 3072;
 constexpr int WN_F32_B = 512;
 constexpr int WN_GBIAS_B = 1024, WN_RBIAS_B = 1536;
@@ -31,7 +24,10 @@
 constexpr int WN_C_R = 16;
 constexpr int WN_C_U = 64;
 constexpr int WN_DBG_ROLES = WN_NT + 3;
-constexpr int WN_C_ONE = WN_NT * WN_TMEM_TILE;
+constexpr int WN_GE = 16;
+constexpr int WN_NTE = 4;
+constexpr int WN_KE = 5;
+constexpr int64_t WN_HAND_MAX_BYTES = 2LL << 30;
 
 
 struct WnHead {
@@ -55,12 +51,16 @@
   int rstride;
   int stream_mode;
   int chunks_per_stream;
+  int kb;
   int join[WN_NT];
   int src_slot[WN_NT];
   int snap_slot[24];
   float det1_b[32], det2_w[64], det2_b[2];
   float* snap;
   int64_t n_rows;
+  float* hand;
+  int64_t n_hand;
+  int hand_rows;
   float* enc_out;
   float* det_out;
   float* post;
```

New measurement: 94.50, median of 6. 3.8% higher.
